# hristo-stripe/pinot

Hardware: AMD Instinct MI355X
Metric: rows/sec for filtered GROUP BY SUM at 1/8 GPUs + achieved HBM GB/s vs peak (higher is better)
Workload: dtype int64; 1 GPU; adanalytics; segments_per_gpu=30, total_rows=1006632960, queries_in_flight=3, parallelism=dp1

## Files before the change

### __graft_entry__.py

```python
from __future__ import annotations

import os
import subprocess
import sys

ROOT = os.path.dirname(os.path.abspath(__file__))
CSRC = os.path.join(ROOT, "pinot_amd", "csrc")
HIPCC = os.environ.get("HIPCC", "/opt/rocm/bin/hipcc")
HIP_FLAGS = ["--offload-arch=gfx950", "-O3", "-std=c++17", "-fPIC", "-munsafe-fp-atomics", "-Wall",
             "-Wno-unused-function", "-Wno-unused-const-variable", "-shared"]

KERNELS = os.path.join(CSRC, "pgpu_kernels.hip")
RUNTIME = os.path.join(CSRC, "pgpu_runtime.cpp")
ITERSTATS = os.path.join(CSRC, "pgpu_iterstats.cpp")
NODE = os.path.join(CSRC, "pgpu_node.cpp")
RAWFWD = os.path.join(CSRC, "pgpu_rawfwd.cpp")
ROARING = os.path.join(CSRC, "pgpu_roaring.cpp")
GDICT = os.path.join(CSRC, "pgpu_gdict.hip")
FOLD = os.path.join(CSRC, "pgpu_fold.hip")
SELECT = os.path.join(CSRC, "pgpu_select.hip")
MODE = os.path.join(CSRC, "pgpu_mode.hip")
PRESENCE = os.path.join(CSRC, "pgpu_presence.hip")
OBJ = os.path.join(ROOT, "build", "obj")
KERNEL_TUS = 6
DEPS = [os.path.join(CSRC, "pgpu_internal.h"), os.path.join(CSRC, "pgpu_host.h"), os.path.join(CSRC, "pgpu_axis.h"),
        os.path.join(CSRC, "pgpu_segplan.h"), os.path.join(ROOT, "include", "pinot_gpu.h")]

LIBS = []
for variant, extra in (("", []), ("_prof", ["-DPGPU_PROFILE_BUILD"])):
    objs = [(os.path.join(OBJ, f"kernels{variant}_tu{k}.o"), KERNELS, extra + [f"-DPGPU_TU={k}"])
            for k in range(KERNEL_TUS)]
    objs.append((os.path.join(OBJ, f"runtime{variant}.o"), RUNTIME, extra))
    objs.append((os.path.join(OBJ, f"iterstats{variant}.o"), ITERSTATS, extra))
    objs.append((os.path.join(OBJ, f"node{variant}.o"), NODE, extra))
    objs.append((os.path.join(OBJ, f"rawfwd{variant}.o"), RAWFWD, extra))
    objs.append((os.path.join(OBJ, f"roaring{variant}.o"), ROARING, extra))
    objs.append((os.path.join(OBJ, f"gdict{variant}.o"), GDICT, extra))
    objs.append((os.path.join(OBJ, f"fold{variant}.o"), FOLD, extra))
    objs.append((os.path.join(OBJ, f"select{variant}.o"), SELECT, extra))
    objs.append((os.path.join(OBJ, f"mode{variant}.o"), MODE, extra))
    objs.append((os.path.join(OBJ, f"presence{variant}.o"), PRESENCE, extra))
    LIBS.append((os.path.join(ROOT, "pinot_amd", f"libpinotgpu{variant}.so"), objs))
LIBS.append((os.path.join(ROOT, "pinot_amd", "libpinotgpu_synth.so"),
             [(os.path.join(OBJ, "synth.o"), os.path.join(CSRC, "synth.hip"), [])]))
ORACLE_LIB = (os.path.join(ROOT, "oracle", "libpinot_cpu.so"), os.path.join(ROOT, "oracle", "pinot_cpu.c"))


def _stale(out: str, srcs) -> bool:
    if not os.path.exists(out):
        return True
    t = os.path.getmtime(out)
    return any(os.path.getmtime(s) > t for s in list(srcs) + DEPS if os.path.exists(s))


def build() -> None:
    from concurrent.futures import ThreadPoolExecutor
    os.makedirs(OBJ, exist_ok=True)
    jobs = []
    libs = [l for l in LIBS if not (os.environ.get("PGPU_SKIP_PROF_BUILD") and "_prof" in l[0])]
    for out, objs in libs:
        for obj, src, extra in objs:
            if _stale(obj, [src]):
                jobs.append([HIPCC] + HIP_FLAGS[:-1] + ["-c"] + extra + [src, "-o", obj])

    def run(cmd):
        print("+", " ".join(cmd), flush=True)
        return subprocess.run(cmd, capture_output=True, text=True)

    workers = max(1, min(8, os.cpu_count() or 1))
    with ThreadPoolExecutor(workers) as pool:
        for cmd, r in zip(jobs, pool.map(run, jobs)):
            if r.returncode != 0:
                sys.stderr.write(r.stdout + r.stderr)
                raise subprocess.CalledProcessError(r.returncode, cmd)
    for out, objs in libs:
        if _stale(out, [o for o, _, _ in objs]):
            cmd = [HIPCC, "--offload-arch=gfx950", "-shared", "-fPIC"] + [o for o, _, _ in objs] + ["-o", out, "-ldl"]
            print("+", " ".join(cmd), flush=True)
            subprocess.run(cmd, check=True)
    out, src = ORACLE_LIB
    if os.path.exists(src) and _stale(out, [src]):
        cmd = ["gcc", "-O3", "-march=x86-64-v2", "-fPIC", "-shared", "-std=c11", "-Wall", "-pthread", src, "-o", out]
        print("+", " ".join(cmd), flush=True)
        subprocess.run(cmd, check=True)
    sys.path.insert(0, ROOT)
    import pinot_amd
    from pinot_amd import _lib
    _lib.load()


def smoke() -> None:
    sys.path.insert(0, ROOT)
    import numpy as np

    from oracle import engine
    from oracle.segment_writer import build_segment
    from pinot_amd._lib import PGPU_INT
    from pinot_amd.plan import GpuPlanMaker
    from pinot_amd.query import parse_sql
    from pinot_amd.segment import GpuContext, GpuSegment

    rng = np.random.default_rng(0)
    n = 100_003
    cols = {"day": (PGPU_INT, rng.integers(0, 64, n, dtype=np.int32) + 17800),
            "acct": (PGPU_INT, rng.integers(0, 5000, n, dtype=np.int32) * 7),
            "clicks": (PGPU_INT, rng.integers(0, 1 << 20, n, dtype=np.int32))}
    seg = build_segment("smoke_0", cols)
    sql = ("SELECT day, SUM(clicks), COUNT(*) FROM t WHERE day BETWEEN 17810 AND 17840 AND acct IN (7, 14, 700) "
           "GROUP BY day ORDER BY SUM(clicks) DESC LIMIT 100")
# ... 21 lines not shown
```

### pinot_amd/csrc/pgpu_internal.h

```cpp
#pragma once
#include <hip/hip_runtime.h>
#include <stdint.h>

#define PGPU_TILE 4096
#define PGPU_WT 2048
#define PGPU_WAVE_TILE PGPU_WT
#define PGPU_THREADS(dense) ((dense) ? 512 : 1024)
#define PGPU_WAVES_OF(dense) (PGPU_THREADS(dense) / 64)
#define PGPU_NLOAD_OF(dense) ((dense) ? 2 : 4)
#define PGPU_NCONS_OF(dense) (PGPU_WAVES_OF(dense) - PGPU_NLOAD_OF(dense))
#define PGPU_MAX_SLOTS 8
#define PGPU_MAX_AGGS 16
#define PGPU_MAX_GCOLS 16
#define PGPU_MAX_STAGE 6
#define PGPU_RING_MAX 64
#define PGPU_CQ_CAP 1024
#define PGPU_CQ_FLUSH 256
#define PGPU_CQ_TILES 32
#define PGPU_AGG_LIST 1024
#define PGPU_DOC_U 4
#define PGPU_LDS_LIMIT 163840
#define PGPU_LDS_TABLE_BYTES (32 * 1024)
#define PGPU_SLICE_RANGES 4
#define PGPU_MAX_STAGE_INSTRS 31
// ... 218 lines not shown
#define PGPU_PART_BITS 21

#define PGPU_MODE_AGG 0
#define PGPU_MODE_LDS 1
#define PGPU_MODE_GLOBAL 2
#define PGPU_MODE_PART 3
#define PGPU_PART_MIN_KEYS 65536
#define PGPU_PART_LDS_BYTES (128 * 1024)
#define PGPU_PART_MAX_PARTS 8192
#define PGPU_PART_MAX_SECTIONS 5
#define PGPU_PSCAN_MAX_PARTS 2048
#define PGPU_MODE_HASH 4
#define PGPU_HASH_EMPTY (~0ull)

__host__ __device__ inline uint32_t pgpu_key_owner_of(const int64_t* key, int kw, int world) {
  uint64_t h = (uint64_t)key[0];
  for (int w = 1; w < kw; ++w) h = h * 0x9E3779B97F4A7C15ull + (uint64_t)key[w];
  h ^= h >> 33;
  h *= 0xff51afd7ed558ccdull;
  h ^= h >> 33;
  return (uint32_t)(h % (uint64_t)world);
}
struct NodeOps {
  int32_t op[PGPU_MAX_SECTIONS];
};

#define PGPU_STAT_MATCHED 0
#define PGPU_STAT_SCANNED 1
#define PGPU_STAT_SECTOR_BYTES 2
#define PGPU_STAT_DENSE_BYTES 3
#define PGPU_NSTATS 4
#define PGPU_SLOT_SKIP 0x40000000
#define PGPU_CANCEL_POLL 16

struct DevParams {
  const DevSeg* segs;
  const DevInstr* instrs;
  const DevColumn* cols;
  const int32_t* pool;
  const int32_t* const* remaps;
  int64_t* table;
  int64_t* slab;
  int64_t* stats;
  int64_t* prof;
  uint64_t G;
  int32_t nseg;
  int32_t total_tiles;
  int32_t ncols;
  int32_t nagg;
  int32_t ngcols;
  int32_t nsec;
  int32_t mode;
  int32_t flags;
  int32_t ring_slots;
  int32_t slot_bytes;
  int32_t inflight;
  int32_t ltab_bytes;
  int32_t max_instrs;
  int32_t dense;
  uint32_t* recs;
  uint32_t* rcount;
  int32_t pshift;
  int32_t nparts;
  int32_t rcap;
  int32_t rw;
  int32_t pcol;
  int32_t rec_idbits;
  const void* pdict;
  int32_t pscan;
  int32_t pscan_wave_bytes;
  int32_t pscan_kb, pscan_vb;
  int32_t mask_rows;
  int32_t cons_bytes;
  int32_t direct;
  int32_t dslots;
  int32_t min_instrs;
  int32_t slice_shift;
  int32_t ldict;
  uint32_t pdict_n;
  const uint32_t* pfor;
  int32_t for_bits;
  int32_t for_nblk;
  uint32_t cancel_gen;
  uint32_t* pcount;
  uint32_t* pcap;
  uint32_t* poff;
  int32_t* p2work;
  uint64_t pblock;
  int32_t psample;
  int32_t p2grid;
  uint32_t* segmask;
  int32_t* hflag;
  uint32_t* leaf_bits;
  uint32_t* segany;
  const int32_t* cancel;
  int32_t key_words;
  int32_t key_split;
  int32_t segmask_rows;
  int32_t cancel_poll;
  int32_t rd_planes;
  int32_t mv_gmask;
  int32_t rd_pfx;
  int32_t rd_skip;
  int32_t rs_vplanes;
  int32_t total_units;
  int32_t rk_leaves;
  int32_t rk_ids;
  const struct InvLeafX* invx;
  const struct DevContainer* rk_ctab;
  const uint32_t* cand_ct;
  uint32_t* fsm_fn;
  int32_t fuse;
  int32_t fuse_nslabs;
  uint32_t* fuse_ticket;
  int64_t* fuse_stats_out;
  uint8_t* fuse_seg_out;
  int64_t* fuse_host_table;
  uint64_t fuse_table_words;
  int64_t* fuse_spare;
  uint64_t gstride64[PGPU_MAX_GCOLS];
  DevAgg aggs[PGPU_MAX_AGGS];
  int32_t gcols[PGPU_MAX_GCOLS];
  uint32_t gstride[PGPU_MAX_GCOLS];
  int32_t sec_op[PGPU_MAX_SECTIONS];
};
static_assert(sizeof(DevParams) <= 4096, "DevParams is a kernel argument");

#define PGPU_FUSE_LDS_BYTES 2064
#define PGPU_FUSE_MAX_TABLE_WORDS 8192

#define PGPU_FLAG_STATS 1
#define PGPU_FLAG_PROFILE 2
#define PGPU_FLAG_NT 4
#define PGPU_NPROF 12
#define PGPU_P_L_TOTAL 0
#define PGPU_P_L_FREE 1
#define PGPU_P_L_PUB 2
#define PGPU_P_L_ISSUE 3
#define PGPU_P_C_TOTAL 4
#define PGPU_P_C_FULL 5
#define PGPU_P_C_FILTER 6
#define PGPU_P_C_AGG 7
#define PGPU_P_C_FLUSH 8
#define PGPU_P_C_TILES 9
#define PGPU_P_C_FETCH 10
#define PGPU_P_C_DECODE 11

inline uint32_t pgpu_lds_fixed_bytes(int dense, int ltab_bytes, int mask_rows) {
  return (uint32_t)(PGPU_FLAG_BYTES + PGPU_NCONS_OF(dense) * PGPU_CONS_BYTES(dense, mask_rows) +
                    ((ltab_bytes + 15) & ~15));
}
inline uint32_t pgpu_lds_bytes(int dense, int ring_slots, int slot_bytes, int ltab_bytes, int mask_rows) {
  return pgpu_lds_fixed_bytes(dense, ltab_bytes, mask_rows) + (uint32_t)(ring_slots * slot_bytes);
}

inline int pgpu_stage_region_bytes(int bits, bool sliced = false) {
  return (bits % 8 == 0 && !sliced) ? 64 * (4 * bits + 16) : 256 * bits;
}
inline int pgpu_stage_instrs(int bits, bool sliced = false) {
  return (bits % 8 == 0 && !sliced) ? bits / 4 + 1 : (bits + 3) / 4;
}

#define PGPU_TK_COUNT 0
#define PGPU_TK_SUM_I64 1
#define PGPU_TK_SUM_SPLIT 2
#define PGPU_TK_SUM_F64 3
// ... 130 lines not shown
```

### pinot_amd/csrc/pgpu_kernels.hip

```cpp
#include <hip/hip_runtime.h>
#include <hip/hip_ext.h>
#include <stdint.h>

#include <algorithm>

#include "../../include/pinot_gpu.h"
#include "pgpu_internal.h"

#ifndef PGPU_TU
#define PGPU_TU -1
#endif
#define PGPU_TU_COMMON 5
#define TU_HAS(k) (PGPU_TU < 0 || PGPU_TU == (k))

#define WT PGPU_WT
#define MAXS PGPU_MAX_SLOTS
#define U PGPU_DOC_U
#define FI __device__ __forceinline__

namespace {

typedef uint32_t u32x4 __attribute__((ext_vector_type(4)));
typedef uint32_t u32x2 __attribute__((ext_vector_type(2)));

#define GAS __attribute__((address_space(1)))
#define LAS __attribute__((address_space(3)))
template <class T>
FI T gld(const T* p, size_t i) { return ((const GAS T*)p)[i]; }
#define CAS __attribute__((address_space(4)))
template <class T>
FI T cld(const T* p) {
  if constexpr (sizeof(T) > 8) {
    static_assert(sizeof(T) % 4 == 0, "dword-sized metadata");
    uint32_t w[sizeof(T) / 4];
#pragma unroll
    for (unsigned i = 0; i < sizeof(T) / 4; ++i) w[i] = ((const CAS uint32_t*)p)[i];
    T v;
    __builtin_memcpy(&v, w, sizeof(T));
    return v;
  } else {
    return *(const CAS T*)p;
  }
}
template <class T>
FI T cld(const T* p, size_t i) { return ((const CAS T*)p)[i]; }
FI int sgpr(int v) { return __builtin_amdgcn_readfirstlane(v); }
#ifdef PGPU_PROFILE_BUILD
struct Prof {
  bool on;
  int64_t t[PGPU_NPROF];
};
FI int64_t now(const Prof& pf) { return pf.on ? (int64_t)__builtin_amdgcn_s_memtime() : 0; }
#define PROF_ADD(pf, k, since) do { if ((pf).on) (pf).t[k] += (int64_t)__builtin_amdgcn_s_memtime() - (since); } while (0)
#define PROF_ON(pf) ((pf).on)
#else
struct Prof {
  static constexpr bool on = false;
  int64_t t[1];
};
FI int64_t now(const Prof&) { return 0; }
#define PROF_ADD(pf, k, since) do { (void)(since); } while (0)
#define PROF_ON(pf) false
#endif
FI uint32_t bswap32(uint32_t x) { return __builtin_bswap32(x); }
FI uint32_t lowmask(uint32_t b) { return 0xFFFFFFFFu >> (32u - b); }
FI uint32_t lane_bit(uint32_t m, int i) { return __builtin_amdgcn_ubfe(m, (uint32_t)i, 1u); }
FI int lane_id() { return threadIdx.x & 63; }

FI void wave_sync() {
  __builtin_amdgcn_fence(__ATOMIC_SEQ_CST, "wavefront");
  __builtin_amdgcn_wave_barrier();
}

FI int64_t wave_sum_i64(int64_t v) {
#pragma unroll
  for (int o = 32; o > 0; o >>= 1) v += __shfl_xor(v, o, 64);
  return v;
}
FI double wave_sum_f64(double v) {
#pragma unroll
  for (int o = 32; o > 0; o >>= 1) v += __shfl_xor(v, o, 64);
  return v;
}
FI int64_t wave_min_i64(int64_t v) {
#pragma unroll
  for (int o = 32; o > 0; o >>= 1) { int64_t t = __shfl_xor(v, o, 64); v = t < v ? t : v; }
  return v;
}
FI int64_t wave_max_i64(int64_t v) {
#pragma unroll
// ... 2417 lines not shown
        __syncthreads();
      }
      if (tid == 0) {
        p.table[col] = red[0];
        if (p.fuse_host_table) p.fuse_host_table[col] = red[0];
      }
    }
  }
  if (tid == 0) *p.fuse_ticket = 0u;
}

#define PGPU_RDIRECT_DEPTH 2
struct RdIssue {
  const uint32_t* sliced;
  int bits;
  int plane0;
  const uint32_t* psliced;
  int pbits;
};
FI void rd_load_issue(const DevParams& p, int seg, RdIssue& is) {
  const DevSeg* sg = p.segs + seg;
  const DevColumn* cols = p.cols + cld(&sg->col_begin);
  const int qc = cld(&sg->stage_col[0]);
  is.sliced = (const uint32_t*)cld(&cols[qc].sliced);
  is.bits = cld(&cols[qc].bits);
  is.plane0 = cld(&sg->f_plane0);
  const int pc = cld(&sg->pfx_col);
  is.psliced = pc >= 0 ? (const uint32_t*)cld(&cols[pc].sliced) : nullptr;
  is.pbits = pc >= 0 ? cld(&cols[pc].bits) : 0;
}
template <int PL>
FI void rd_load_tile(const RdIssue& is, int tile_in_seg, uint32_t (&x)[PL]) {
  const uint32_t* src = is.sliced + ((size_t)tile_in_seg * is.bits + is.plane0) * 64 + lane_id();
  const int np = is.bits - is.plane0;
#pragma unroll
  for (int k = 0; k < PL; ++k)
    x[k] = k < np ? __builtin_nontemporal_load(src + 64 * k) : 0u;
}
template <int PK>
FI void rd_load_prefix(const RdIssue& is, int tile_in_seg, uint32_t (&y)[PK]) {
  const uint32_t* src = is.psliced + ((size_t)tile_in_seg * is.pbits + (is.pbits - PK)) * 64 + lane_id();
#pragma unroll
  for (int k = 0; k < PK; ++k) y[k] = __builtin_nontemporal_load(src + 64 * k);
}
template <int PL>
FI uint32_t rd_lt(const uint32_t (&x)[PL], uint32_t c) {
  uint32_t br = 0;
#pragma unroll
  for (int k = 0; k < PL; ++k)
    br = __builtin_amdgcn_bitop3_b32((uint32_t)-(int32_t)((c >> k) & 1u), x[k], br, 0xB2);
  return (c >> PL) ? ~0u : br;
}
template <int PL>
FI uint32_t rd_filter(const SegState& ss, const uint32_t (&x)[PL], uint32_t valid,
                      uint32_t& lane_scanned) {
  if (!(ss.f_kind[0] >> 8)) lane_scanned += __popc(valid);
  uint32_t m = rd_lt(x, ss.f_r0hi[0]) & ~rd_lt(x, ss.f_r0lo[0]);
  for (int r = 1; r < ss.f_nr[0]; ++r) {
    const uint32_t lo = cld(&ss.sg->f_rng[0][r][0]), hi = cld(&ss.sg->f_rng[0][r][1]);
    m |= rd_lt(x, hi) & ~rd_lt(x, lo);
  }
  return valid & (ss.f_sneg[0] ? ~m : m);
}
template <int PK>
FI uint32_t rd_prefix(const SegState& ss, const uint32_t (&y)[PK], uint32_t mm, uint32_t& lane_scanned) {
  uint32_t pm = 0;
  const int nr = cld(&ss.sg->pfx_nr);
  for (int r = 0; r < nr; ++r) {
    const uint32_t lo = cld(&ss.sg->pfx_rng[r][0]), hi = cld(&ss.sg->pfx_rng[r][1]);
    pm |= rd_lt(y, hi) & ~rd_lt(y, lo);
  }
  lane_scanned += __popc(mm & ~pm);
  return mm & pm;
}

template <int S>
struct RdSlot {
  static constexpr int value = S;
};
struct RdSkip {
  int seg, tb, nt;
  int a, b;
  int cw0;
  uint32_t kw;
  uint64_t live;
};
FI void rd_skip_enter(const DevParams& p, RdSkip& g, int seg, int t0, int tend) {
  g.seg = seg;
  g.tb = cld(&p.segs[seg].tile_begin);
  g.nt = cld(&p.segs[seg].ntiles);
  g.a = max(t0 - g.tb, 0);
  g.b = min(tend - g.tb, g.nt);
  g.cw0 = (g.a >> 5) - p.rd_skip;
  g.kw = 0u;
  g.live = 0ull;
}
template <int NW>
FI void rd_skip_chunk(const DevParams& p, RdSkip& g, int cidx, int t0, int64_t& dense_bytes) {
  static_assert(NW == 4, "a wave's tiles are every 4th bit of a keep word");
  const DevSeg* sg = p.segs + g.seg;
  const int wi = g.cw0 + lane_id(), s = g.a - 32 * wi, e = g.b - 32 * wi;
  const uint32_t range = (e <= 0 || s >= 32 || lane_id() >= p.rd_skip) ? 0u
                         : ((e >= 32 ? ~0u : ((1u << e) - 1u)) & (s <= 0 ? ~0u : ~((1u << s) - 1u)));
  uint32_t kw = range & (0x11111111u << ((cidx + t0 - g.tb) & 3));
  const uint32_t* rows = (const uint32_t*)cld(&sg->skip_rows);
  if (rows) {
    const int n = cld(&sg->skip_n), wpr = cld(&sg->skip_wpr);
    const uint32_t wic = (uint32_t)(wi < wpr ? wi : wpr - 1);
    static_assert(PGPU_SLICE_RANGES % 2 == 0, "ids are probed in pairs");
    uint32_t keep = 0u;
    if (kw != 0u) {
      for (int i0 = 0; i0 < n; i0 += 2) {
        uint32_t v[2][PGPU_PRESENCE_PROBES];
#pragma unroll
        for (int i = 0; i < 2; ++i) {
          const int id = i0 + i < n ? i0 + i : 0;
          const uint32_t r01 = cld((const uint32_t*)&sg->skip_row[id][0]);
          const uint32_t r23 = cld((const uint32_t*)&sg->skip_row[id][2]);
          v[i][0] = (rows + (size_t)(r01 & 0xFFFFu) * wpr)[wic];
          v[i][1] = (rows + (size_t)(r01 >> 16) * wpr)[wic];
          v[i][2] = (rows + (size_t)(r23 & 0xFFFFu) * wpr)[wic];
          v[i][3] = (rows + (size_t)(r23 >> 16) * wpr)[wic];
        }
        keep |= (v[0][0] & v[0][1] & v[0][2] & v[0][3]) | (v[1][0] & v[1][1] & v[1][2] & v[1][3]);
      }
    }
    kw &= wi < wpr ? keep : 0u;
    if ((p.flags & PGPU_FLAG_STATS) && lane_id() == 0) {
      const int w0 = max(g.cw0, g.a >> 5), w1 = min(g.cw0 + p.rd_skip - 1, (g.b - 1) >> 5);
      if (w1 >= w0) dense_bytes += (int64_t)(w1 - w0 + 1) * n * PGPU_PRESENCE_PROBES * 4;
    }
  }
  g.kw = kw;
  g.live = __builtin_amdgcn_ballot_w64(kw != 0u);
}
template <int NW>
FI bool rd_skip_next(const DevParams& p, RdSkip& g, int cidx, int t0, int tend, int& seg, int& tile_in_seg,
                     int64_t& dense_bytes) {
  for (;;) {
    if (g.live) {
      const int l = __builtin_ctzll(g.live);
      const uint32_t w = (uint32_t)__builtin_amdgcn_readlane((int)g.kw, l);
      if (lane_id() == l) g.kw &= g.kw - 1u;
      if ((w & (w - 1u)) == 0u) g.live &= g.live - 1ull;
      seg = g.seg;
      tile_in_seg = ((g.cw0 + l) << 5) + __builtin_ctz(w);
      return true;
    }
    g.cw0 += p.rd_skip;
    if ((g.cw0 << 5) >= g.b) {
      if (g.tb + g.nt >= tend || g.seg + 1 >= p.nseg) return false;
      rd_skip_enter(p, g, g.seg + 1, t0, tend);
      g.cw0 += p.rd_skip;
      if ((g.cw0 << 5) >= g.b) continue;
    }
    rd_skip_chunk<NW>(p, g, cidx, t0, dense_bytes);
  }
}

template <int MODE, int PL, int PK, bool SK>
FI Stats rdirect_consumer(const DevParams& p, const Lds& L, int cidx, int t0, int ntiles, Prof& pf) {
  constexpr int NW = PGPU_DIRECT_WAVES, RD = PGPU_RDIRECT_DEPTH;
  const int64_t t_start = now(pf);
  const int lane = lane_id();
  Cons cv;
  {
    unsigned char* base = L.cons + (size_t)cidx * p.cons_bytes;
    cv.masks = (uint32_t*)base;
    cv.queue = (uint16_t*)(base + p.mask_rows * 256);
    cv.klist = (int32_t*)(base + p.mask_rows * 256);
    cv.vlist = cv.klist + PGPU_AGG_LIST;
    cv.acc = (int64_t*)(base + p.mask_rows * 256 + PGPU_CONS_LIST_BYTES_OF(0));
    cv.qtiles = (int32_t*)(base + p.mask_rows * 256 + PGPU_CONS_LIST_BYTES_OF(0) + PGPU_CONS_ACC_BYTES);
  }
  if (MODE == PGPU_MODE_AGG && lane < PGPU_MAX_AGGS) cv.acc[lane] = lane < p.nagg ? sec_identity(p.aggs[lane].op) : 0;
  wave_sync();
  int64_t matched = 0, scanned = 0, sector_bytes = 0, dense_bytes = 0;
  uint32_t lane_scanned = 0, lane_matched = 0;
  LaneAcc la;
#pragma unroll
  for (int k = 0; k < NREG_ACC; ++k) la.v[k] = k < p.nagg ? sec_identity(p.aggs[k].op) : 0;
  int qn = 0, qt = 0;
  SegState ss;
  int cseg = -1;
  if constexpr (SK) {
    if (ntiles > 0) {
      const int tend = t0 + ntiles;
      RdSkip g;
      rd_skip_enter(p, g, cursor_at(p, t0).seg, t0, tend);
      RdIssue is;
      int iseg = -1;
      uint32_t x[RD][PL];
      uint32_t y[RD][PK > 0 ? PK : 1];
      int kseg[RD], ktile[RD];
      bool kv[RD];
#pragma unroll
      for (int s = 0; s < RD; ++s) {
        kseg[s] = ktile[s] = 0;
        kv[s] = rd_skip_next<NW>(p, g, cidx, t0, tend, kseg[s], ktile[s], dense_bytes);
        if (kv[s]) {
          if (kseg[s] != iseg) rd_load_issue(p, iseg = kseg[s], is);
          rd_load_tile(is, ktile[s], x[s]);
          if constexpr (PK > 0) rd_load_prefix<PK>(is, ktile[s], y[s]);
        }
      }
      int poll = p.cancel_poll;
      bool stop = false;
      auto turn = [&](auto slot) -> bool {
          constexpr int s = decltype(slot)::value;
          if (!kv[s]) return false;
          if (--poll == 0) {
            poll = p.cancel_poll;
            if (query_cancelled(p)) {
              stop = true;
              return false;
            }
          }
          const int tseg = kseg[s], ttile = ktile[s];
          if (qn && (qn >= PGPU_CQ_FLUSH || qt >= PGPU_CQ_TILES || tseg != cseg)) {
            const int64_t tq = now(pf);
            flush_queue<MODE, NW>(p, L, cv, la, ss, qn, matched, scanned, sector_bytes, dense_bytes, pf);
            PROF_ADD(pf, PGPU_P_C_FLUSH, tq);
            qn = qt = 0;
          }
          if (tseg != cseg) {
            cseg = tseg;
            load_seg(p, cseg, ss);
          }
          const int64_t tf = now(pf);
#ifdef PGPU_PROFILE_BUILD
          if (pf.on) pf.t[PGPU_P_C_TILES] += 1;
#endif
          const int doc0 = ttile * WT;
          uint32_t valid;
          {
            const int ndocs = min(WT, ss.num_docs - doc0);
            const int rem = ndocs - 32 * lane;
            valid = rem >= 32 ? 0xFFFFFFFFu : (rem <= 0 ? 0u : ((1u << rem) - 1u));
            if ((p.flags & PGPU_FLAG_STATS) && lane == 0)
              dense_bytes += ((int64_t)ndocs * (ss.f_bits[0] - cld(&ss.sg->f_plane0) + PK) + 7) / 8;
          }
          uint32_t mm = rd_filter(ss, x[s], valid, lane_scanned);
          if constexpr (PK > 0) mm = rd_prefix<PK>(ss, y[s], mm, lane_scanned);
          kv[s] = rd_skip_next<NW>(p, g, cidx, t0, tend, kseg[s], ktile[s], dense_bytes);
          if (kv[s]) {
            if (kseg[s] != iseg) rd_load_issue(p, iseg = kseg[s], is);
            rd_load_tile(is, ktile[s], x[s]);
            if constexpr (PK > 0) rd_load_prefix<PK>(is, ktile[s], y[s]);
          }
          PROF_ADD(pf, PGPU_P_C_FILTER, tf);
          const int64_t ta = now(pf);
          direct_candidates<MODE, NW>(p, L, cv, la, ss, ttile, mm, qn, qt, lane_matched, matched, scanned, sector_bytes,
                                      dense_bytes, pf);
          PROF_ADD(pf, PGPU_P_C_AGG, ta);
          return true;
      };
      static_assert(RD == 2, "the ring's turns are written out");
      while (turn(RdSlot<0>{}) && turn(RdSlot<1>{})) {
      }
      if (qn && !stop) flush_queue<MODE, NW>(p, L, cv, la, ss, qn, matched, scanned, sector_bytes, dense_bytes, pf);
    }
  } else if (cidx < ntiles) {
    const int own = (ntiles - cidx + NW - 1) / NW;
    Cursor ci = cursor_at(p, t0 + cidx), cur = ci;
    RdIssue is;
    rd_load_issue(p, ci.seg, is);
    uint32_t x[RD][PL];
    uint32_t y[RD][PK > 0 ? PK : 1];
#pragma unroll
    for (int s = 0; s < RD; ++s) {
      if (s < own) {
        if (s > 0 && cursor_advance(p, ci, NW)) rd_load_issue(p, ci.seg, is);
        rd_load_tile(is, ci.tile_in_seg, x[s]);
        if constexpr (PK > 0) rd_load_prefix<PK>(is, ci.tile_in_seg, y[s]);
      }
    }
    int poll = p.cancel_poll;
    bool stop = false;
    for (int k0 = 0; k0 < own && !stop; k0 += RD) {
#pragma unroll
      for (int s = 0; s < RD; ++s) {
        const int k = k0 + s;
        if (k >= own || stop) break;
        if (--poll == 0) {
          poll = p.cancel_poll;
          if (query_cancelled(p)) {
            stop = true;
            break;
          }
        }
        if (k > 0) cursor_advance(p, cur, NW);
        if (qn && (qn >= PGPU_CQ_FLUSH || qt >= PGPU_CQ_TILES || cur.seg != cseg)) {
          const int64_t tq = now(pf);
          flush_queue<MODE, NW>(p, L, cv, la, ss, qn, matched, scanned, sector_bytes, dense_bytes, pf);
          PROF_ADD(pf, PGPU_P_C_FLUSH, tq);
          qn = qt = 0;
        }
        if (cur.seg != cseg) {
          cseg = cur.seg;
          load_seg(p, cseg, ss);
        }
        const int64_t tf = now(pf);
#ifdef PGPU_PROFILE_BUILD
        if (pf.on) pf.t[PGPU_P_C_TILES] += 1;
#endif
        const int doc0 = cur.tile_in_seg * WT;
        uint32_t valid;
        {
          const int ndocs = min(WT, ss.num_docs - doc0);
          const int rem = ndocs - 32 * lane;
          valid = rem >= 32 ? 0xFFFFFFFFu : (rem <= 0 ? 0u : ((1u << rem) - 1u));
          if ((p.flags & PGPU_FLAG_STATS) && lane == 0)
            dense_bytes += ((int64_t)ndocs * (ss.f_bits[0] - cld(&ss.sg->f_plane0) + PK) + 7) / 8;
        }
        uint32_t mm = rd_filter(ss, x[s], valid, lane_scanned);
        if constexpr (PK > 0) mm = rd_prefix<PK>(ss, y[s], mm, lane_scanned);
        if (k + RD < own) {
          if (cursor_advance(p, ci, NW)) rd_load_issue(p, ci.seg, is);
          rd_load_tile(is, ci.tile_in_seg, x[s]);
          if constexpr (PK > 0) rd_load_prefix<PK>(is, ci.tile_in_seg, y[s]);
        }
        PROF_ADD(pf, PGPU_P_C_FILTER, tf);
        const int64_t ta = now(pf);
        direct_candidates<MODE, NW>(p, L, cv, la, ss, cur.tile_in_seg, mm, qn, qt, lane_matched, matched, scanned,
                                    sector_bytes, dense_bytes, pf);
        PROF_ADD(pf, PGPU_P_C_AGG, ta);
      }
    }
    if (qn && !stop) flush_queue<MODE, NW>(p, L, cv, la, ss, qn, matched, scanned, sector_bytes, dense_bytes, pf);
// ... 3225 lines not shown
```

### pinot_amd/csrc/pgpu_runtime.cpp

```cpp
#include <hip/hip_runtime.h>

#include <algorithm>
#include <atomic>
#include <chrono>
#include <cmath>
#include <cstdarg>
#include <cstdio>
#include <cstdlib>
#include <cstring>
#include <memory>
#include <mutex>
#include <string>
#include <thread>
#include <vector>

#include "../../include/pinot_gpu.h"
#include "pgpu_host.h"
#include "pgpu_internal.h"
#include "pgpu_segplan.h"

hipError_t pgpu_prepare_query_kernels(size_t lds_bytes);
hipError_t pgpu_launch_table_init(const DevParams& p, hipStream_t st);
hipError_t pgpu_launch_query(const DevParams& p, int grid, size_t dyn_smem, hipStream_t st);
hipError_t pgpu_launch_query_direct(const DevParams& p, int grid, size_t dyn_smem, hipStream_t st,
// ... 3475 lines not shown
    const HostColumn* h = v.host(qc);
    if (!h->presence || h->presence->state.load(std::memory_order_acquire) == PresenceState::kDeclined) continue;
    const double keep = presence_keep(v.dev(qc)->card, nruns);
    if (out->h && keep >= out->keep) continue;
    out->h = h;
    out->col = qc;
    out->n = nruns;
    for (int i = 0; i < out->n; ++i) out->ids[i] = (uint32_t)runs[i].a;
    out->keep = keep;
  }
  return out->h != nullptr;
}

struct PresenceScratch {
  std::vector<SkipChoice> ch;
  std::vector<double> saved;
  std::vector<const uint32_t*> rows;
  std::vector<int32_t> wpr;
};
PresenceScratch& presence_scratch() {
  static thread_local PresenceScratch s;
  return s;
}

void plan_presence(const pgpu_query_desc* q, Packer& pk, DevParams& p, LaunchPlan& pl, SkipInfo* si, bool* settled) {
  *settled = true;
  const int after = pk.env.presence_after;
  const int64_t thr = pk.env.presence_switch_bytes;
  if (p.direct != PGPU_KV_RDIRECT || (q->flags & PGPU_Q_EXACT_FILTER_STATS) || after < 0 || thr < 0) return;
  if (!pgpu_rd_skip_ok(p.rd_planes, p.rd_pfx)) return;
  const int nseg = (int)pk.segs.size();
  PlanScratch& sc = plan_scratch();
  PresenceScratch& ps = presence_scratch();
  std::vector<SkipChoice>& ch = ps.ch;
  std::vector<double>& saved = ps.saved;
  ch.assign((size_t)nseg, SkipChoice());
  saved.assign((size_t)nseg, 0.0);
  double want = 0;
  for (int s = 0; s < nseg; ++s) {
    const pgpu_segment_plan& sp = q->segments[s];
    const DevSeg& ds = pk.segs[s];
    if (ds.ntiles <= 0 || ds.nstage < 1) continue;
    SegView v{q, &sp, sp.segment, sp.filter, sp.num_filter_nodes};
    if (!skip_choice(v, sc.analysis(v, s), &ch[s])) continue;
    const DevColumn& lc = pk.cols[ds.col_begin + ds.stage_col[0]];
    const double bpt = 256.0 * (lc.bits - ds.f_plane0 + p.rd_pfx);
    saved[s] = presence_saved(ch[s].keep, ch[s].n, ds.ntiles, bpt);
    if (saved[s] > 0) want += saved[s];
    else ch[s].h = nullptr;
  }
  if (!pgpu_lead_switch(want, thr)) return;
  double have = 0;
  std::vector<const uint32_t*>& rows = ps.rows;
  std::vector<int32_t>& wpr = ps.wpr;
  rows.assign((size_t)nseg, nullptr);
  wpr.assign((size_t)nseg, 0);
  int ncand = 0, nready = 0, ndeclined = 0;
  for (int s = 0; s < nseg; ++s) {
    if (!ch[s].h) continue;
    PresenceState* st = ch[s].h->presence.get();
    if (st->state.load(std::memory_order_acquire) == PresenceState::kNone && st->wanted.fetch_add(1) + 1 >= after)
      pl.presence_builds.push_back(ch[s].h->presence);
    rows[s] = presence_ready(*ch[s].h, &wpr[s]);
    if (rows[s]) have += saved[s];
    ++ncand;
    nready += rows[s] != nullptr;
    ndeclined += !rows[s] && st->state.load(std::memory_order_acquire) == PresenceState::kDeclined;
  }
  *settled = pl.presence_builds.empty() && (nready == ncand || ndeclined == ncand);
  if (!pgpu_lead_switch(have, thr)) return;
  for (int s = 0; s < nseg; ++s) {
    if (!rows[s]) continue;
    DevSeg& ds = pk.segs[s];
    ds.skip_rows = rows[s];
    ds.skip_wpr = wpr[s];
    ds.skip_n = ch[s].n;
    for (int i = 0; i < ch[s].n; ++i)
      for (int j = 0; j < PGPU_PRESENCE_PROBES; ++j) ds.skip_row[i][j] = (uint16_t)pgpu_presence_row_of(ch[s].ids[i], j);
    if (!si->on) si->col = ch[s].col, si->ids = ch[s].n, si->keep = ch[s].keep;
    si->on = true;
  }
  const int cw = pk.env.presence_chunk_words;
  p.rd_skip = std::min(64, std::max(1, cw));
}

int pack_and_plan(pgpu_context* ctx, const pgpu_query_desc* q, const pgpu_table_layout& L, Packer& pk, DevParams& p,
                  LaunchPlan& pl, const PlanEnv* given_env = nullptr, bool* settled = nullptr) {
  LeadInfo li;
  PlanEnv env;
  if (given_env) env = *given_env;
  else env.read();
  for (int attempt = 0; attempt < 2; ++attempt) {
    pk.clear();
    pk.env = env;
    pl = LaunchPlan();
    li.allow = attempt == 0;
    const double tp0 = HostTiming::us();
    int rc = pack_query(ctx, q, L, pk, p, &li);
    host_timing().add(2, tp0, HostTiming::us());
    if (rc == kLeadRetry && attempt == 0) continue;
    if (rc) return rc;
    const double tl0 = HostTiming::us();
    drop_reference_replay(q, pk);
    rc = plan_launch(ctx->num_cus, q, L, pk, p, pl);
    host_timing().add(HostTiming::kPlanLaunch, tl0, HostTiming::us());
    if (rc) return rc;
    if (!li.switched || p.direct == PGPU_KV_RDIRECT) break;
  }
  SkipInfo si;
  const double ts0 = HostTiming::us();
  bool presence_settled = true;
  plan_presence(q, pk, p, pl, &si, &presence_settled);
  if (settled) *settled = presence_settled;
  host_timing().add(HostTiming::kPresence, ts0, HostTiming::us());
  if (plan_trace_on()) trace_plan(pk, p, pl, li, si);
  return PGPU_OK;
}

hipError_t create_query_streams(pgpu_context* ctx) {
  hipError_t e = ctx->qstream ? hipSuccess : hipStreamCreateWithFlags(&ctx->qstream, hipStreamNonBlocking);
  if (e == hipSuccess && !ctx->qstream2) e = hipStreamCreateWithFlags(&ctx->qstream2, hipStreamNonBlocking);
  return e;
}

int query_stream(pgpu_context* ctx, void* stream, hipStream_t* out) {
  std::lock_guard<std::mutex> lk(ctx->mu);
  if (!stream) {
    const hipError_t ce = create_query_streams(ctx);
    if (ce != hipSuccess) return fail(PGPU_E_HIP, "query stream: %s", hipGetErrorString(ce));
  }
  if (!ctx->cstream) {
    const hipError_t ce = hipStreamCreateWithFlags(&ctx->cstream, hipStreamNonBlocking);
    if (ce != hipSuccess) return fail(PGPU_E_HIP, "cancel stream: %s", hipGetErrorString(ce));
  }
  *out = stream ? (hipStream_t)stream : ctx->qstream;
  return PGPU_OK;
}

struct StreamPick {
  hipStream_t st = nullptr;
  int index = -1;
  hipEvent_t ev0 = nullptr, ev1 = nullptr;
  hipEvent_t done = nullptr;
  uint64_t seq = 0, prev_seq = 0;
};

bool fuse_ext_events() {
  static const bool ext = !env_flag("PGPU_FUSE_EVENT_PACKETS");
  return ext;
}

int pick_stream(pgpu_context* ctx, void* stream, bool fused, Workspace* ws, StreamPick* k) {
  static const bool one_stream = env_int("PGPU_QUERY_STREAMS") == 1;
  k->ev0 = ws->ev0;
  k->ev1 = ws->ev1;
  k->done = ws->done;
  const int rc = query_stream(ctx, stream, &k->st);
  if (rc || stream) return rc;
  hipEvent_t wait_for = nullptr;
  {
    std::lock_guard<std::mutex> lk(ctx->mu);
    k->index = fused && !one_stream && ctx->last_fused_stream == 0 ? 1 : 0;
    if (k->index) k->st = ctx->qstream2;
    const uint64_t seq = ++ctx->submit_seq;
    if (fused) {
      ctx->last_fused_stream = k->index;
// ... 734 lines not shown
        hipEventElapsedTime(&since, s.ev1, qq->ev1) == hipSuccess)
      ms = std::max(0.f, std::min(ms, since));
  }
  qq->stats.kernel_ms = ms;
  qq->stats.kernel_variant = qq->params.pscan ? PGPU_KV_PSCAN : qq->params.direct;
  if (const int st = qq->stop.load()) {
    if (out_stats) *out_stats = qq->stats;
    return fail(st, st == PGPU_E_TIMEOUT ? "query passed its deadline before it finished (EXECUTION_TIMEOUT_ERROR)"
                                         : "query cancelled");
  }
  if (qq->exact_fsm) {
    const int64_t* ent = (const int64_t*)qq->ws->h_fsment.p;
    int64_t total = 0;
    for (int i = 0; i < qq->params.nseg; ++i) total += ent[i];
    qq->stats.num_entries_scanned_in_filter = total;
    qq->stats.filter_stats_exact = 1;
  }
  if (qq->exact_filter) {
    const uint32_t* bits = (const uint32_t*)qq->ws->h_leafbits.p;
    const size_t nr = qq->replay.size();
    std::vector<int64_t> counts(nr, 0);
    std::atomic<size_t> next{0};
    auto work = [&]() {
      for (size_t i = next++; i < nr; i = next++) {
        const pgpu_query::FilterReplay& r = qq->replay[i];
        std::vector<const uint32_t*> leaf(r.num_leaves);
        for (int k = 0; k < r.num_leaves; ++k) leaf[k] = bits + r.bits_off + (int64_t)k * r.ntiles * 64;
        counts[i] = reference_entries_scanned(r.nodes.data(), (int)r.nodes.size(), leaf.data(), r.num_leaves,
                                              r.num_docs, r.leaf_off.empty() ? nullptr : r.leaf_off.data());
      }
    };
    const size_t nthreads = std::min<size_t>({nr, 16, std::max(1u, std::thread::hardware_concurrency() / 2)});
    std::vector<std::thread> pool;
    for (size_t t = 1; t < nthreads; ++t) pool.emplace_back(work);
    work();
    for (std::thread& t : pool) t.join();
    int64_t total = 0;
    for (int64_t c : counts) {
      if (c < 0) return fail(PGPU_E_INVALID, "filter program cannot be replayed for statistics");
      total += c;
    }
    qq->stats.num_entries_scanned_in_filter = total;
    qq->stats.filter_stats_exact = 1;
  }
  if (qq->params.mode == PGPU_MODE_HASH) {
    int32_t flag = 0;
    memcpy(&flag, (const char*)qq->ws->h_stats.p + 8 * PGPU_NSTATS, 4);
    if (flag) {
      if (out_stats) *out_stats = qq->stats;
      if (!qq->tracked.empty())
        return fail(PGPU_E_GROUPS_LIMIT, "hash group-by table overflow: a segment meets more distinct group keys than "
                    "numGroupsLimit %lld (the reference keeps the first-seen keys only)", (long long)qq->groups_limit);
      return fail(PGPU_E_UNSUPPORTED, "hash group-by table overflow (more distinct keys than the holder limits allow)");
    }
    const int64_t* cnt = (const int64_t*)qq->ws->h_segcnt.p;
    for (size_t i = 0; i < qq->tracked.size(); ++i)
      if (cnt[i] >= qq->groups_limit) qq->stats.num_groups_limit_reached = 1;
    for (size_t i = 0; i < qq->tracked.size(); ++i)
      if (cnt[i] > qq->groups_limit && qq->tracked_map[i]) {
        if (out_stats) *out_stats = qq->stats;
        return fail(PGPU_E_GROUPS_LIMIT,
                    "segment %d meets %lld distinct group keys > numGroupsLimit %lld: the reference keeps the "
                    "first-seen keys only (DictionaryBasedGroupKeyGenerator)",
                    qq->tracked[i], (long long)cnt[i], (long long)qq->groups_limit);
      }
  }
  if (qq->params.flags & PGPU_FLAG_PROFILE) {
    const int nw = qq->grid * (qq->params.direct != PGPU_KV_RING || qq->params.pscan ? 4 : PGPU_WAVES_OF(qq->params.dense));
    std::vector<int64_t> pr((size_t)nw * PGPU_NPROF);
    HIP_TRY(hipMemcpy(pr.data(), qq->params.prof, pr.size() * 8, hipMemcpyDeviceToHost));
    double sum[PGPU_NPROF] = {0};
    int nl = 0, nc = 0;
    for (int w = 0; w < nw; ++w) {
      const bool ld = qq->params.direct == PGPU_KV_RING && !qq->params.pscan &&
                      (w % PGPU_WAVES_OF(qq->params.dense)) < PGPU_NLOAD_OF(qq->params.dense);
      ld ? ++nl : ++nc;
      for (int k = 0; k < PGPU_NPROF; ++k) sum[k] += (double)pr[(size_t)w * PGPU_NPROF + k];
    }
    fprintf(stderr,
            "[pgpu profile] kernel %.3f ms | loader/wave: total %.0f free %.0f pub %.0f issue %.0f | consumer/wave: "
            "total %.0f full %.0f filter %.0f (fetch %.0f decode %.0f) agg %.0f flush %.0f tiles %.1f\n",
            ms, sum[0] / nl, sum[1] / nl, sum[2] / nl, sum[3] / nl, sum[4] / nc, sum[5] / nc, sum[6] / nc,
            sum[10] / nc, sum[11] / nc, sum[7] / nc, sum[8] / nc, sum[9] / nc);
  }
  if (out_stats) *out_stats = qq->stats;
  return PGPU_OK;
}

int pgpu_query_release(pgpu_query* qq) {
  if (!qq) return PGPU_OK;
  if (qq->done) (void)hipEventSynchronize(qq->done);
  else (void)hipStreamSynchronize(qq->stream);
  if (qq->tws) release_ws(qq->ctx, qq->tws);
  release_ws(qq->ctx, qq->ws);
  if (qq->seq) {
    StreamPick k;
    k.seq = qq->seq;
    release_ev_slot(qq->ctx, k);
  }
  delete qq;
  return PGPU_OK;
}

}

namespace {

int topk_spec(const pgpu_table_layout* L, const pgpu_topk* o, TopkDev* out) {
  TopkDev t{};
  t.G = L->num_keys;
  t.nsec = L->num_sections;
  t.kw = L->key_kind == PGPU_KEYS_HASH ? L->key_words : 0;
  t.desc = o->descending ? 1 : 0;
  t.key_base = o->key_base;
  if (o->source == PGPU_TOPK_AGG) {
    const int a = o->agg_index;
    if (a < 0 || a >= 16) return fail(PGPU_E_INVALID, "top-k aggregation index %d", a);
    const int sec = L->agg_section[a];
    t.sec = sec;
    const bool split = L->agg_sum_parts[a] > 1;
    const int op = L->section_op[sec];
    const int vt = L->agg_value_type[a];
    t.fxe = split && (vt == PGPU_FLOAT || vt == PGPU_DOUBLE) ? L->agg_sum_exp[a] : 0;
    t.parts = split ? L->agg_sum_parts[a] : 1;
    switch (o->agg_fn) {
      case PGPU_AGG_COUNT: t.mode = PGPU_TK_COUNT; break;
      case PGPU_AGG_SUM:
        t.mode = op == PGPU_RED_SUM_F64 ? PGPU_TK_SUM_F64 : (split ? PGPU_TK_SUM_SPLIT : PGPU_TK_SUM_I64);
        break;
      case PGPU_AGG_AVG:
        t.mode = op == PGPU_RED_SUM_F64 ? PGPU_TK_AVG_F64 : (split ? PGPU_TK_AVG_SPLIT : PGPU_TK_AVG_I64);
        break;
      case PGPU_AGG_MIN:
      case PGPU_AGG_MAX:
        t.mode = (vt == PGPU_INT || vt == PGPU_LONG) ? PGPU_TK_MINMAX_INT : PGPU_TK_MINMAX_FP;
        break;
      default: return fail(PGPU_E_INVALID, "top-k aggregation fn %d", o->agg_fn);
    }
    if (o->agg_fn != PGPU_AGG_COUNT && sec <= 0) return fail(PGPU_E_INVALID, "top-k aggregation %d has no section", a);
  } else if (o->source == PGPU_TOPK_GROUP) {
    const int g = o->group_index, n = o->num_group_columns;
    if (g < 0 || g >= n || !o->group_cardinalities) return fail(PGPU_E_INVALID, "top-k group column %d", g);
    const int split = t.kw == 2 ? L->key_split : n;
    t.word = g < split ? 0 : 1;
    uint64_t st = 1;
    for (int j = t.word == 0 ? 0 : split; j < g; ++j) st *= (uint64_t)std::max(1, o->group_cardinalities[j]);
    t.stride = st;
    t.card = (uint64_t)std::max(1, o->group_cardinalities[g]);
    t.mode = PGPU_TK_GROUP;
  } else {
    return fail(PGPU_E_INVALID, "top-k source %d", o->source);
  }
  *out = t;
  return PGPU_OK;
}

int compact_into(pgpu_context* ctx, Workspace* ws, const pgpu_table_layout* L, const void* dev_table,
                 hipStream_t st, int64_t* out_keys, int64_t* out_cells, uint64_t capacity,
                 uint64_t* out_num_groups, const pgpu_topk* order = nullptr) {
  const uint64_t G = L->num_keys;
  const int nsec = L->num_sections;
  const int kw = L->key_kind == PGPU_KEYS_HASH ? L->key_words : 0;
  const int okw = kw > 1 ? kw : 1;
  const uint64_t nb = (G + 4095) / 4096;
  HIP_TRY(ws->cmp_counts.ensure(4 * nb + 16, ctx->mpool, st));
  HIP_TRY(ws->cmp_total.ensure(16, ctx->mpool, st));
// ... 1259 lines not shown
```

Baseline: 22920 billion rows/s.

## Deal surviving skip tiles round-robin across waves by rank instead of fixed stride

Before, each of the four waves took every fourth tile position of a keep word. Now the surviving tiles are ranked with a wave-wide prefix scan and dealt round-robin across waves using a bit-parallel mod-4 prefix count. This aims to balance load when presence skipping leaves uneven survivors. It also caches skip row pointers per segment, issues segment loads on entry, and computes the starting segment by division when all segments have equal tile counts. A profiling dump path is added as well. The extra scan and readlane run on every chunk.

```diff
diff --git a/__graft_entry__.py b/__graft_entry__.py
--- a/__graft_entry__.py
+++ b/__graft_entry__.py
@@ -24,7 +24,8 @@
 OBJ = os.path.join(ROOT, "build", "obj")
 KERNEL_TUS = 6
 DEPS = [os.path.join(CSRC, "pgpu_internal.h"), os.path.join(CSRC, "pgpu_host.h"), os.path.join(CSRC, "pgpu_axis.h"),
-        os.path.join(CSRC, "pgpu_segplan.h"), os.path.join(ROOT, "include", "pinot_gpu.h")]
+        os.path.join(CSRC, "pgpu_segplan.h"), os.path.join(CSRC, "pgpu_skip_stripe.h"),
+        os.path.join(ROOT, "include", "pinot_gpu.h")]
 
 LIBS = []
 for variant, extra in (("", []), ("_prof", ["-DPGPU_PROFILE_BUILD"])):
diff --git a/pinot_amd/csrc/pgpu_internal.h b/pinot_amd/csrc/pgpu_internal.h
--- a/pinot_amd/csrc/pgpu_internal.h
+++ b/pinot_amd/csrc/pgpu_internal.h
@@ -324,6 +324,7 @@
   int32_t for_bits;
   int32_t for_nblk;
   uint32_t cancel_gen;
+  int32_t rd_seg_tiles;
   uint32_t* pcount;
   uint32_t* pcap;
   uint32_t* poff;
diff --git a/pinot_amd/csrc/pgpu_kernels.hip b/pinot_amd/csrc/pgpu_kernels.hip
--- a/pinot_amd/csrc/pgpu_kernels.hip
+++ b/pinot_amd/csrc/pgpu_kernels.hip
@@ -6,6 +6,7 @@
 
 #include "../../include/pinot_gpu.h"
 #include "pgpu_internal.h"
+#include "pgpu_skip_stripe.h"
 
 #ifndef PGPU_TU
 #define PGPU_TU -1
@@ -2589,13 +2590,21 @@
   int seg, tb, nt;
   int a, b;
   int cw0;
+  int rank;
+  const uint32_t* rows;
+  int n, wpr;
   uint32_t kw;
   uint64_t live;
 };
-FI void rd_skip_enter(const DevParams& p, RdSkip& g, int seg, int t0, int tend) {
+FI void rd_skip_enter(const DevParams& p, RdSkip& g, RdIssue& is, int seg, int t0, int tend) {
+  const DevSeg* sg = p.segs + seg;
   g.seg = seg;
-  g.tb = cld(&p.segs[seg].tile_begin);
-  g.nt = cld(&p.segs[seg].ntiles);
+  g.tb = cld(&sg->tile_begin);
+  g.nt = cld(&sg->ntiles);
+  g.rows = (const uint32_t*)cld(&sg->skip_rows);
+  g.n = cld(&sg->skip_n);
+  g.wpr = cld(&sg->skip_wpr);
+  rd_load_issue(p, seg, is);
   g.a = max(t0 - g.tb, 0);
   g.b = min(tend - g.tb, g.nt);
   g.cw0 = (g.a >> 5) - p.rd_skip;
@@ -2603,16 +2612,15 @@
   g.live = 0ull;
 }
 template <int NW>
-FI void rd_skip_chunk(const DevParams& p, RdSkip& g, int cidx, int t0, int64_t& dense_bytes) {
-  static_assert(NW == 4, "a wave's tiles are every 4th bit of a keep word");
+FI void rd_skip_chunk(const DevParams& p, RdSkip& g, int cidx, int64_t& dense_bytes) {
+  static_assert(NW == PGPU_SKIP_STRIPE_WAVES, "pgpu_skip_stripe deals to four waves");
   const DevSeg* sg = p.segs + g.seg;
   const int wi = g.cw0 + lane_id(), s = g.a - 32 * wi, e = g.b - 32 * wi;
-  const uint32_t range = (e <= 0 || s >= 32 || lane_id() >= p.rd_skip) ? 0u
-                         : ((e >= 32 ? ~0u : ((1u << e) - 1u)) & (s <= 0 ? ~0u : ~((1u << s) - 1u)));
-  uint32_t kw = range & (0x11111111u << ((cidx + t0 - g.tb) & 3));
-  const uint32_t* rows = (const uint32_t*)cld(&sg->skip_rows);
+  uint32_t kw = (e <= 0 || s >= 32 || lane_id() >= p.rd_skip) ? 0u
+                : ((e >= 32 ? ~0u : ((1u << e) - 1u)) & (s <= 0 ? ~0u : ~((1u << s) - 1u)));
+  const uint32_t* rows = g.rows;
   if (rows) {
-    const int n = cld(&sg->skip_n), wpr = cld(&sg->skip_wpr);
+    const int n = g.n, wpr = g.wpr;
     const uint32_t wic = (uint32_t)(wi < wpr ? wi : wpr - 1);
     static_assert(PGPU_SLICE_RANGES % 2 == 0, "ids are probed in pairs");
     uint32_t keep = 0u;
@@ -2638,12 +2646,15 @@
       if (w1 >= w0) dense_bytes += (int64_t)(w1 - w0 + 1) * n * PGPU_PRESENCE_PROBES * 4;
     }
   }
-  g.kw = kw;
-  g.live = __builtin_amdgcn_ballot_w64(kw != 0u);
+  const int nk = __popc(kw), before = wave_excl_scan(nk);
+  int cnt;
+  g.kw = pgpu_skip_stripe(kw, (uint32_t)(g.rank + before), cidx, &cnt);
+  g.rank += __builtin_amdgcn_readlane(before + nk, 63);
+  g.live = __builtin_amdgcn_ballot_w64(g.kw != 0u);
 }
 template <int NW>
-FI bool rd_skip_next(const DevParams& p, RdSkip& g, int cidx, int t0, int tend, int& seg, int& tile_in_seg,
-                     int64_t& dense_bytes) {
+FI bool rd_skip_next(const DevParams& p, RdSkip& g, RdIssue& is, int cidx, int t0, int tend, int& seg,
+                     int& tile_in_seg, int64_t& dense_bytes) {
   for (;;) {
     if (g.live) {
       const int l = __builtin_ctzll(g.live);
@@ -2657,11 +2668,11 @@
     g.cw0 += p.rd_skip;
     if ((g.cw0 << 5) >= g.b) {
       if (g.tb + g.nt >= tend || g.seg + 1 >= p.nseg) return false;
-      rd_skip_enter(p, g, g.seg + 1, t0, tend);
+      rd_skip_enter(p, g, is, g.seg + 1, t0, tend);
       g.cw0 += p.rd_skip;
       if ((g.cw0 << 5) >= g.b) continue;
     }
-    rd_skip_chunk<NW>(p, g, cidx, t0, dense_bytes);
+    rd_skip_chunk<NW>(p, g, cidx, dense_bytes);
   }
 }
 
@@ -2694,9 +2705,9 @@
     if (ntiles > 0) {
       const int tend = t0 + ntiles;
       RdSkip g;
-      rd_skip_enter(p, g, cursor_at(p, t0).seg, t0, tend);
       RdIssue is;
-      int iseg = -1;
+      g.rank = 0;
+      rd_skip_enter(p, g, is, p.rd_seg_tiles ? t0 / p.rd_seg_tiles : cursor_at(p, t0).seg, t0, tend);
       uint32_t x[RD][PL];
       uint32_t y[RD][PK > 0 ? PK : 1];
       int kseg[RD], ktile[RD];
@@ -2704,9 +2715,8 @@
 #pragma unroll
       for (int s = 0; s < RD; ++s) {
         kseg[s] = ktile[s] = 0;
-        kv[s] = rd_skip_next<NW>(p, g, cidx, t0, tend, kseg[s], ktile[s], dense_bytes);
+        kv[s] = rd_skip_next<NW>(p, g, is, cidx, t0, tend, kseg[s], ktile[s], dense_bytes);
         if (kv[s]) {
-          if (kseg[s] != iseg) rd_load_issue(p, iseg = kseg[s], is);
           rd_load_tile(is, ktile[s], x[s]);
           if constexpr (PK > 0) rd_load_prefix<PK>(is, ktile[s], y[s]);
         }
@@ -2749,9 +2759,8 @@
           }
           uint32_t mm = rd_filter(ss, x[s], valid, lane_scanned);
           if constexpr (PK > 0) mm = rd_prefix<PK>(ss, y[s], mm, lane_scanned);
-          kv[s] = rd_skip_next<NW>(p, g, cidx, t0, tend, kseg[s], ktile[s], dense_bytes);
+          kv[s] = rd_skip_next<NW>(p, g, is, cidx, t0, tend, kseg[s], ktile[s], dense_bytes);
           if (kv[s]) {
-            if (kseg[s] != iseg) rd_load_issue(p, iseg = kseg[s], is);
             rd_load_tile(is, ktile[s], x[s]);
             if constexpr (PK > 0) rd_load_prefix<PK>(is, ktile[s], y[s]);
           }
diff --git a/pinot_amd/csrc/pgpu_runtime.cpp b/pinot_amd/csrc/pgpu_runtime.cpp
--- a/pinot_amd/csrc/pgpu_runtime.cpp
+++ b/pinot_amd/csrc/pgpu_runtime.cpp
@@ -3581,6 +3581,10 @@
   }
   const int cw = pk.env.presence_chunk_words;
   p.rd_skip = std::min(64, std::max(1, cw));
+  int32_t common = nseg > 0 ? pk.segs[0].ntiles : 0;
+  for (int s = 1; s < nseg; ++s)
+    if (pk.segs[s].ntiles != common) common = 0;
+  p.rd_seg_tiles = common > 0 ? common : 0;
 }
 
 int pack_and_plan(pgpu_context* ctx, const pgpu_query_desc* q, const pgpu_table_layout& L, Packer& pk, DevParams& p,
@@ -4481,6 +4485,18 @@
             "total %.0f full %.0f filter %.0f (fetch %.0f decode %.0f) agg %.0f flush %.0f tiles %.1f\n",
             ms, sum[0] / nl, sum[1] / nl, sum[2] / nl, sum[3] / nl, sum[4] / nc, sum[5] / nc, sum[6] / nc,
             sum[10] / nc, sum[11] / nc, sum[7] / nc, sum[8] / nc, sum[9] / nc);
+    if (const char* path = getenv("PGPU_PROFILE_DUMP")) {
+      if (FILE* f = fopen(path, "a")) {
+        fprintf(f, "# query grid %d waves %d kernel_ms %.4f: wave total full filter agg flush tiles\n", qq->grid, nw, ms);
+        for (int w = 0; w < nw; ++w) {
+          const int64_t* r = &pr[(size_t)w * PGPU_NPROF];
+          fprintf(f, "%d %lld %lld %lld %lld %lld %lld\n", w, (long long)r[PGPU_P_C_TOTAL], (long long)r[PGPU_P_C_FULL],
+                  (long long)r[PGPU_P_C_FILTER], (long long)r[PGPU_P_C_AGG], (long long)r[PGPU_P_C_FLUSH],
+                  (long long)r[PGPU_P_C_TILES]);
+        }
+        fclose(f);
+      }
+    }
   }
   if (out_stats) *out_stats = qq->stats;
   return PGPU_OK;
diff --git a/pinot_amd/csrc/pgpu_skip_stripe.h b/pinot_amd/csrc/pgpu_skip_stripe.h
--- /dev/null
+++ b/pinot_amd/csrc/pgpu_skip_stripe.h
@@ -0,0 +1,29 @@
+#pragma once
+#include <stdint.h>
+
+#ifndef __host__
+#define PGPU_SKIP_STRIPE_HD
+#else
+#define PGPU_SKIP_STRIPE_HD __host__ __device__
+#endif
+
+#define PGPU_SKIP_STRIPE_WAVES 4
+
+PGPU_SKIP_STRIPE_HD inline uint32_t pgpu_skip_stripe(uint32_t w, uint32_t first, int wave, int* count) {
+  uint32_t c0 = w, c1 = 0u;
+#define PGPU_SKIP_STRIPE_STEP(s)                         \
+  {                                                      \
+    const uint32_t d0 = c0 << (s), d1 = c1 << (s);       \
+    c1 ^= d1 ^ (c0 & d0);                                \
+    c0 ^= d0;                                            \
+  }
+  PGPU_SKIP_STRIPE_STEP(1)
+  PGPU_SKIP_STRIPE_STEP(2)
+  PGPU_SKIP_STRIPE_STEP(4)
+  PGPU_SKIP_STRIPE_STEP(8)
+  PGPU_SKIP_STRIPE_STEP(16)
+#undef PGPU_SKIP_STRIPE_STEP
+  const uint32_t t = ((uint32_t)wave - first + 1u) & 3u;
+  *count = __builtin_popcount(w);
+  return w & ((t & 1u) ? c0 : ~c0) & ((t & 2u) ? c1 : ~c1);
+}
```

New measurement: 20600 billion rows/s. 0.899x the previous value.
